# flanglet/kanzi-cpp

Hardware: AMD Instinct MI355X
Metric: encode+decode MB/s on the synthetic stand-in for silesia.tar (bit-exact) (higher is better)
Workload: dtype u8

## Files before the change

kanzi-cpp_amd/csrc/bwt_fwd.hip:

```cpp
#include "common.hpp"
#include "stages.hpp"
#include "bwt_common.hpp"

#include <cstdlib>
#include <cstring>
#include <algorithm>
#include <cmath>
#include "prims.hpp"
#include <chrono>
#include <vector>

namespace knz {

constexpr u32 SM_TS = 1792;
constexpr u32 SM_WIN = 2048;
constexpr u32 SM_G = 256;
constexpr u32 MED_CAP = 8192;
constexpr u32 SUPER_CAP = 8192;
constexpr int GATHER_THREADS = 512;
constexpr u32 GATHER_ROWS = 16;
static_assert(MED_CAP <= GATHER_ROWS * GATHER_THREADS, "k_bwt_f_gather_desc judges a medium group from one batch of loads");
constexpr u32 LARGE_OS_MIN = 1000000;
constexpr u32 NO_BIT = 0x7FFFFFFFu;

struct FwdView {
    const u32* base;
    int nBlocks;
    u32 total;
    u32* SA;
    u32* ISA;
    u64* ISA2;
    u32 round;
// ... 10 lines not shown

constexpr u32 VERDICT_WHOLE = 1, VERDICT_PLAIN = 2;
__host__ __device__ __forceinline__ u32 verdict_word(u32 round, u32 status, u32 members) { return (round << 24) | (status << 16) | members; }
static_assert(MED_CAP < (1u << 16), "verdict_word keeps a medium group's size in 16 bits");

enum FwdCounter : u32 {
    CNT_SMALL_LEFT = 0,
    CNT_MED = 1,
    CNT_LARGE = 2,
    CNT_LARGE_MEMBERS = 3,
    CNT_RUN = 4,
    CNT_RUN_MEMBERS = 5,
    CNT_RUN_LONGEST = 6,
    CNT_SUPER = 7,
    CNT_RUNS = 8,
    CNT_STAT_SMALL = 10,
    CNT_STAT_SMALL_GROUPS = 11,
    CNT_STAT_MED = 12,
    CNT_TIED = 13,
    CNT_PROBE_CAND = 14,
    CNT_LINKED = 14,
    CNT_LINK_TIED = 15,
    CNT_STAT_MED_GROUPS = 16,
    CNT_STAT_UNSPLIT = 17,
    CNT_STAT_UNSPLIT_MEMBERS = 18,
    CNT_STAT_MAJ = 19,
    CNT_STAT_MAJ_MEMBERS = 20,
    CNT_STAT_ASLEEP = 21,
    CNT_STAT_ASLEEP_MEMBERS = 22,
    CNT_ROUND_SLOTS = 24,
// ... 1114 lines not shown
        const u32 lab = (size <= SM_G) ? hdSlot : ((oldLab >= hdSlot && oldLab < hdSlot + size) ? oldLab : hdSlot + (size >> 1));
        (void)relO;
        const u32 gp = L.oV[t];
        v.SA[slot] = gp;
        if (lab != oldLab) lab_set(v, gp, L.blkBase, lab, oldLab);
        if (t == hd) {
            if (hdSlot != gs) atomicOr(&v.gnew[hdSlot >> 5], 1u << (hdSlot & 31));
            if (size > SM_G) v.medStage[hdSlot >> 8] = make_uint2(hdSlot, size);
            else if (size > 1) surv = 1;
        }
    }
    if (__ballot(surv != 0) != 0 && (tid & 63) == 0) v.counters[CNT_SMALL_LEFT] = 1;
}

template <int THREADS, int ROWS, bool STATS>
__global__ __launch_bounds__(THREADS, (THREADS >= 1024 ? 4 : THREADS / 128)) void k_bwt_f_sort_medium(FwdView v, const uint2* __restrict__ desc, u32 nDesc, int npass, u32 minLen,
                                                               uint2* __restrict__ medNext, uint2* __restrict__ largeNext, const uint2* __restrict__ descInfo,
                                                               uint4* __restrict__ superList)
{
    constexpr int WAVES = THREADS / 64;
    constexpr u32 CAP = (u32)ROWS * THREADS;
    __shared__ MedLds<THREADS, ROWS> L;
    const int tid = (int)threadIdx.x, lane = tid & 63, wave = tid >> 6;
    const unsigned long long ltMask = (lane == 0) ? 0ull : (~0ull >> (64 - lane));

    for (u32 g = blockIdx.x; g < nDesc; g += gridDim.x) {
        const uint2 d = desc[g];
        const u32 gs = d.x, n = d.y;
        if (n <= minLen || n > CAP) continue;
        const uint2 info = descInfo[g];
        {
            u32 k[ROWS], p[ROWS];
#pragma unroll
            for (int r = 0; r < ROWS; r++) { const u32 i = (u32)tid + (u32)r * THREADS; k[r] = 0; p[r] = 0; if (i < n) { k[r] = v.K[gs + i]; p[r] = v.SA[gs + i]; } }
#pragma unroll
            for (int r = 0; r < ROWS; r++) { const u32 i = (u32)tid + (u32)r * THREADS; if (i < n) { L.oK[i] = k[r]; L.oV[i] = p[r]; } }
        }
        __syncthreads();
        if (tid == 0) { L.oldLab = info.y; L.blkBase = info.x; }
        const u32 ka = L.oK[n >> 2], kb = L.oK[n >> 1], kc = L.oK[(n >> 2) * 3];
        const u32 m = (ka == kc) ? ka : kb;
        u32 c = 0;
        for (u32 i = (u32)tid; i < n; i += THREADS) c += (L.oK[i] == m) ? 1u : 0u;
        c = med_block_sum(L, c);
        if (c < n && 2 * c >= n && n <= SUPER_CAP && m == info.y - info.x + 1u) {
            if (tid == 0) { const u32 at = atomicAdd(&v.counters[CNT_SUPER], 1u); superList[at] = make_uint4(gs, n, info.x, info.y); }
            __syncthreads();
            continue;
        }
        if (STATS && tid == 0 && c == n) { atomicAdd(&v.counters[CNT_STAT_UNSPLIT], 1u); atomicAdd(&v.counters[CNT_STAT_UNSPLIT_MEMBERS], n); }
        if (c < n) {
            if (2 * c >= n) {
                const int R = (int)((n + THREADS - 1) / THREADS);
                const u32 waveBase = (u32)wave * (u32)R * 64u;
                u32 key[ROWS], val[ROWS], pos[ROWS];
                u32 runO = 0, runE = 0;
#pragma unroll
                for (int r = 0; r < ROWS; r++) {
                    key[r] = m; val[r] = 0; pos[r] = 0xFFFFFFFFu;
                    if (r < R) {
                        const u32 idx = waveBase + (u32)r * 64u + (u32)lane;
                        const bool valid = idx < n;
                        if (valid) { key[r] = L.oK[idx]; val[r] = L.oV[idx]; }
                        const bool oth = valid && key[r] != m, same = valid && key[r] == m;
                        const unsigned long long bo = __ballot(oth), be = __ballot(same);
                        if (oth) pos[r] = runO + (u32)__popcll(bo & ltMask);
                        if (same) pos[r] = 0x80000000u | (runE + (u32)__popcll(be & ltMask));
                        runO += (u32)__popcll(bo);
                        runE += (u32)__popcll(be);
                    }
                }
                if (lane == 0) { L.wtot[wave] = runO; L.wtot2[wave] = runE; }
                __syncthreads();
                u32 baseO = 0, baseE = 0, nOth = 0;
                for (int w = 0; w < WAVES; w++) { if (w < wave) { baseO += L.wtot[w]; baseE += L.wtot2[w]; } nOth += L.wtot[w]; }
#pragma unroll
                for (int r = 0; r < ROWS; r++) {
                    if (r < R && pos[r] != 0xFFFFFFFFu) {
                        const u32 at = (pos[r] & 0x80000000u) ? (nOth + baseE + (pos[r] & 0x7FFFFFFFu)) : (baseO + pos[r]);
                        L.oK[at] = key[r];
                        L.oV[at] = val[r];
                    }
                }
                __syncthreads();
                if (nOth <= (u32)THREADS) {
                    u32 kk = 0, vv = 0, at = 0;
                    if ((u32)tid < nOth) {
                        kk = L.oK[tid]; vv = L.oV[tid];
                        for (u32 j = 0; j < nOth; j++) { const u32 kj = L.oK[j]; at += (kj < kk || (kj == kk && j < (u32)tid)) ? 1u : 0u; }
                    }
                    __syncthreads();
                    if ((u32)tid < nOth) { L.oK[at] = kk; L.oV[at] = vv; }
                    __syncthreads();
                    u32 lessQ = 0;
                    if ((u32)tid < nOth) lessQ = (L.oK[tid] < m) ? 1u : 0u;
                    lessQ = med_block_sum(L, lessQ);
                    if (tid == 0) { L.oldLab = info.y; L.blkBase = info.x; if (STATS) { atomicAdd(&v.counters[CNT_STAT_MAJ], 1u); atomicAdd(&v.counters[CNT_STAT_MAJ_MEMBERS], n); } }
                    __syncthreads();
                    med_majority_write_back<THREADS, ROWS>(L, v, gs, n, nOth, c, lessQ, m);
                    __syncthreads();
                    continue;
                } else {
                    med_radix_sort<THREADS, ROWS>(L, nOth, npass);
                }
                u32 less = 0;
                for (u32 i = (u32)tid; i < nOth; i += THREADS) less += (L.oK[i] < m) ? 1u : 0u;
                less = med_block_sum(L, less);
#pragma unroll
                for (int k = 0; k < ROWS; k++) {
                    const u32 i = (u32)tid + (u32)k * THREADS;
                    if (i < n) { key[k] = L.oK[i]; val[k] = L.oV[i]; }
                }
                __syncthreads();
#pragma unroll
                for (int k = 0; k < ROWS; k++) {
                    const u32 i = (u32)tid + (u32)k * THREADS;
                    if (i < n) {
                        const u32 at = (i < less) ? i : (i < nOth ? i + c : less + (i - nOth));
                        L.oK[at] = key[k];
                        L.oV[at] = val[k];
                    }
                }
                __syncthreads();
            } else {
                med_radix_sort<THREADS, ROWS>(L, n, npass);
            }
        }
        med_write_back<THREADS, ROWS>(L, v, gs, n, medNext, largeNext);
        __syncthreads();
    }
}

__global__ __launch_bounds__(1024) void k_bwt_f_super(FwdView v, const uint4* __restrict__ superList, u32 h, int npass, uint2* __restrict__ medNext, uint2* __restrict__ largeNext)
{
    constexpr int THREADS = 1024, ROWS = 8;
    constexpr u32 CAP = (u32)ROWS * THREADS;
    __shared__ MedLds<THREADS, ROWS> L;
    __shared__ u16 nxt[CAP];
    __shared__ u16 cn[CAP];
    __shared__ u16 trEnd[CAP];
    __shared__ u32 sEnds;
    __shared__ u32 sMoved[2];
    __shared__ u32 sCmax;
    const int tid = (int)threadIdx.x, lane = tid & 63;
// ... 667 lines not shown
        const u32 step = ((u32)chunks * st == n) ? st : st + 1;
        const u32 logNbChunks = (u32)ilog2_u32((u32)chunks);
        d[0] = (u8)((logNbChunks << 2) | (pIndexSize - 1));
        u32 idx = 1;
        for (int k = 0; k < chunks; k++) {
            const u32 prim = lab_cur(fv, bb + (u32)k * step, bb) - bb;
            for (int sh = (int)(pIndexSize - 1) * 8; sh >= 0; sh -= 8) d[idx++] = (u8)(prim >> sh);
        }
        newLen[b] = hdr + n;
    }
}

__global__ __launch_bounds__(256) void k_bwt_f_med_flags(const uint2* __restrict__ stage, u32 nSlots, u32* __restrict__ flags)
{
    const u32 i = blockIdx.x * 256 + threadIdx.x;
    if (i < nSlots) flags[i] = stage[i].y ? 1u : 0u;
}

__global__ __launch_bounds__(256) void k_bwt_f_med_compact(uint2* __restrict__ stage, u32 nSlots, const u32* __restrict__ prefix, uint2* __restrict__ medNext)
{
    const u32 i = blockIdx.x * 256 + threadIdx.x;
    if (i >= nSlots) return;
    const uint2 d = stage[i];
    if (d.y) { medNext[prefix[i]] = d; stage[i] = make_uint2(0u, 0u); }
}

struct FwdTuning { int nsym; int noRunRound; int runFallback; int stats; int link; int plainLabels; int noPack; int noUnsplitSkip; int noGroupSleep; };
static FwdTuning& fwd_tuning()
{
    static FwdTuning t = [] {
        FwdTuning x; x.nsym = 0; x.noRunRound = 0; x.runFallback = 0; x.stats = 0; x.link = 1; x.plainLabels = 0; x.noPack = 0; x.noUnsplitSkip = 0; x.noGroupSleep = 0;
        if (getenv("KNZ_BWT_PLAIN_LABELS")) x.plainLabels = 1;
        if (getenv("KNZ_BWT_NO_PACK")) x.noPack = 1;
        if (getenv("KNZ_BWT_NO_UNSPLIT_SKIP")) x.noUnsplitSkip = 1;
        if (getenv("KNZ_BWT_NO_GROUP_SLEEP")) x.noGroupSleep = 1;
        if (const char* e = getenv("KNZ_BWT_LINK")) x.link = atoi(e);
        if (getenv("KNZ_BWT_STATS")) x.stats = 1;
        if (const char* e = getenv("KNZ_BWT_NSYM")) x.nsym = atoi(e);
        if (getenv("KNZ_BWT_NO_RUN_ROUND")) x.noRunRound = 1;
        if (getenv("KNZ_BWT_RUN_FALLBACK")) x.runFallback = 1;
        return x;
    }();
    return t;
}
int bwt_forward_tune(const char* key, int value)
{
    FwdTuning& t = fwd_tuning();
    if (!strcmp(key, "rs_onesweep")) { prims::rs_onesweep_knob().store(value); return 0; }
    if (!strcmp(key, "bwt_nsym")) t.nsym = value;
    else if (!strcmp(key, "bwt_no_run_round")) t.noRunRound = value;
    else if (!strcmp(key, "bwt_run_fallback")) t.runFallback = value;
    else if (!strcmp(key, "bwt_stats")) t.stats = value;
    else if (!strcmp(key, "bwt_link")) t.link = value;
    else if (!strcmp(key, "bwt_plain_labels")) t.plainLabels = value;
    else if (!strcmp(key, "bwt_no_pack")) t.noPack = value;
    else if (!strcmp(key, "bwt_no_unsplit_skip")) t.noUnsplitSkip = value;
    else if (!strcmp(key, "bwt_no_group_sleep")) t.noGroupSleep = value;
    else return -1;
    return 0;
}

struct FwdScratch {
    u64* keysA; u64* keysB;
    u32* valsA; u32* valsB;
    u32* SA; u32* ISA; u32* K; u64* ISA2;
    u32* t0; u32* t1; u32* t2; u32* t3;
    u32* gbits; u32* gnew; u32* rtbits; u32* ovr; size_t gbitsWords;
    uint2* med[2]; uint2* medStage; uint2* medVerdict[2]; u32* medFlags; u32* medPrefix; size_t medSlots; uint2* descInfo; uint2* large[2]; uint2* runList; uint4* superList; u32* ebits;
    u32* loff; u32* lbase;
    u32* survTile;
    u32* linkedTile;
    u32* base;
    u32* counters;
    u32* seg2;
    void* scanTmp;
    void* rsMem;
    u32* byteHist;
    u32* classTab; u32* rbits; u32* rcount; u32* rprefix;
    u32* runPos; u32* runE; u32* runL; u32* sE; u32* rcnt; u32* moff;
    u64* runKeysA; u64* runKeysB; u64* sKey;
    size_t maxRuns;
};

// ... 4 lines not shown
    u8* q = p;
    auto take = [&](size_t sz) { u8* r = q; q += fwd_align(sz); return r; };
    const size_t maxMed = 2 * (total / (SM_G + 1) + 2), maxLarge = total / (MED_CAP + 1) + 2;
    w->gbitsWords = ((total + 64) / 64 + SM_WIN / 64 + 4) * 2 + 128;
    w->keysA = (u64*)take(8 * total); w->keysB = (u64*)take(8 * total);
    w->valsA = (u32*)take(4 * total); w->valsB = (u32*)take(4 * total);
    w->SA = (u32*)take(4 * total); w->ISA = (u32*)take(4 * total); w->K = (u32*)take(4 * total);
    w->ISA2 = (VS <= (1u << LAB_BITS)) ? (u64*)take(8 * total) : (u64*)nullptr;
    w->t0 = (u32*)take(4 * total); w->t1 = (u32*)take(4 * total); w->t2 = (u32*)take(4 * total); w->t3 = (u32*)take(4 * total);
    w->gbits = (u32*)take(4 * w->gbitsWords);
    w->gnew = (u32*)take(4 * w->gbitsWords);
    w->rtbits = (u32*)take(4 * w->gbitsWords);
    w->ovr = (u32*)take(4 * total);
    w->med[0] = (uint2*)take(8 * maxMed); w->med[1] = (uint2*)take(8 * maxMed);
    w->medSlots = total / 256 + 2;
    w->medStage = (uint2*)take(8 * w->medSlots); w->medFlags = (u32*)take(4 * w->medSlots + 64); w->medPrefix = (u32*)take(4 * w->medSlots + 64);
    w->medVerdict[0] = (uint2*)take(16 * w->medSlots); w->medVerdict[1] = w->medVerdict[0] + w->medSlots;
    w->large[0] = (uint2*)take(8 * maxLarge); w->large[1] = (uint2*)take(8 * maxLarge);
    w->runList = (uint2*)take(8 * maxMed);
    w->superList = (uint4*)take(16 * maxMed);
    w->descInfo = (uint2*)take(8 * maxMed);
    w->ebits = (u32*)take(4 * w->gbitsWords);
    w->loff = (u32*)take(4 * (maxMed + 1));
    w->lbase = (u32*)take(4 * (maxMed + 1));
    w->survTile = (u32*)take(4 * (total / SM_TS + 64));
    w->linkedTile = (u32*)take(4 * (total / SM_TS + 64));
    w->base = (u32*)take(4ull * (nBlocks + 2));
    w->counters = (u32*)take(256);
    w->byteHist = (u32*)take(1024ull * (nBlocks + 1));
    w->seg2 = (u32*)take(64);
    w->scanTmp = take(prims::scan_tmp_bytes(total + 16));
// ... 33 lines not shown
        if (mode == UNTRIED && survMembers >= total / 8) { mode = TRIAL; trials++; return true; }
        if (mode == ON && survMembers >= total / 64) { mode = APPLIED; return true; }
        return false;
    }
};

struct FwdSort {
    hipStream_t s; const XfStage& st; u32* hp;
    const FwdTuning tune = fwd_tuning();
    BwtView bv; FwdView v; FwdScratch w; size_t maxTotal;
    prims::RsWs rs1;
    u32 total, medSlots, nTiles; int nsym, pbits, kbits;
    bool groupSleep = false;
    u32 h = 1; int cur = 0;
    u64 *keysFree, *keysFree2;
    u32 nRun, runElems, surv, nMed, nLarge, largeElems, survMembers;
    LinkPlan link; LinkTrial linkTr; std::chrono::steady_clock::time_point statT;
    int fetch(u32 first, u32 n) { return hipMemcpyAsync(hp + first, w.counters + first, 4 * (size_t)n, hipMemcpyDeviceToHost, s) == hipSuccess && hipStreamSynchronize(s) == hipSuccess ? 0 : -1; }
    void merge_bits() { hipLaunchKernelGGL(k_bwt_f_merge_bits, GRID1(total / 32 + 2), w.gbits, w.gnew, total / 32 + 2); }
    void enable_run_tiebits() { if (!v.rtbits) { hipMemsetAsync(w.rtbits, 0, 4 * w.gbitsWords, s); v.ovr = w.ovr; v.rtbits = w.rtbits; } }
    void compact_medium(uint2* dst)
    {
        KScope ks_("k_bwt_f_med_compact");
        hipLaunchKernelGGL(k_bwt_f_med_flags, GRID1(medSlots), w.medStage, medSlots, w.medFlags);
        prims::launch_scan<prims::SCAN_SUM_EXCL>(s, w.medFlags, w.medPrefix, medSlots, nullptr, w.scanTmp, w.counters + CNT_MED);
        hipLaunchKernelGGL(k_bwt_f_med_compact, GRID1(medSlots), w.medStage, medSlots, w.medPrefix, dst);
    }
    void bounds(u32 n, bool last, const u32* bits = nullptr, u32 len = 0, u32 wordsPerWin = 0)
    {
        if (bits) { KScope ks_("k_bwt_f_r0_winsum"); hipLaunchKernelGGL(k_bwt_f_r0_winsum, GRID1(n), bits, len, n, w.t0, w.t2, wordsPerWin); }
        if (last) { KScope ks_("k_bwt_f_scan_max"); prims::launch_scan<prims::SCAN_MAX_INCL>(s, w.t0, w.t1, n, nullptr, w.scanTmp); }
        KScope ks_("k_bwt_f_scan_min"); prims::launch_scan<prims::SCAN_MIN_INCL>(s, w.t2, w.t3, n, nullptr, w.scanTmp);
    }
    template <class KEY, bool HAS_VAL> int sort_one_segment(u32 n, KEY* ka, KEY* kb, u32* va, u32* vb, int loBit, int hiBit, bool oneRead = true)
    {
        hipLaunchKernelGGL(prims::k_rs_one_segment, dim3(1), dim3(64), 0, s, w.seg2, n);
        prims::rs_launch_layout(s, rs1);
        return prims::rs_sort<KEY, HAS_VAL>(s, rs1, ka, kb, va, vb, (size_t)n, loBit, hiBit, oneRead);
    }
    int setup(void* scratch, size_t scratchBytes, BwtSuffixArrays* sa)
    {
// ... 4 lines not shown
        hipMemsetAsync(st.newLen, 0, sizeof(u32) * st.nBlocks, s);
        { KScope ks_("k_bwt_f_r0_hist");
          hipMemsetAsync(w.byteHist, 0, 1024ull * st.nBlocks, s);
          hipLaunchKernelGGL(k_bwt_f_bytehist, dim3(64, (unsigned)st.nBlocks), dim3(256), 0, s, bv, w.base, w.byteHist);
          hipLaunchKernelGGL(k_bwt_f_choose_nsym, dim3(1), dim3(256), 0, s, w.byteHist, st.nBlocks, w.counters + CNT_LONGEST_BLOCK, w.counters + CNT_NSYM); }
        if (hipMemcpyAsync(hp, w.base + st.nBlocks, 4, hipMemcpyDeviceToHost, s) != hipSuccess || fetch(CNT_LONGEST_BLOCK, 2)) return -1;
        total = hp[0];
        if (sa) { sa->SA = w.SA; sa->base = w.base; sa->total = total; }
        if (total == 0) return 0;
        v.base = w.base; v.nBlocks = st.nBlocks; v.total = total; v.SA = w.SA; v.ISA = w.ISA; v.K = w.K; v.ISA2 = (w.ISA2 != nullptr && !tune.plainLabels) ? w.ISA2 : (u64*)nullptr;
        v.round = 0; v.gbits = w.gbits; v.gnew = w.gnew; v.counters = w.counters; v.medStage = w.medStage; v.ovr = nullptr; v.rtbits = nullptr;
        v.verdictNow = nullptr; v.verdictWas = nullptr;
        medSlots = (u32)((size_t)total / 256 + 1); nTiles = (total + SM_TS - 1) / SM_TS;
        survMembers = total;
        hipMemsetAsync(w.medStage, 0, 8ull * w.medSlots, s);
        groupSleep = !tune.noUnsplitSkip && !tune.noGroupSleep;
        if (groupSleep) hipMemsetAsync(w.medVerdict[0], 0, 16ull * w.medSlots, s);
        pbits = bits_for(hp[CNT_LONGEST_BLOCK], 1);
        const int fit = (64 - pbits) / 8, want = (hp[CNT_NSYM] == 5u) ? 5 : 4;
        nsym = fit < want ? fit : want;
        if (tune.nsym >= 1) nsym = tune.nsym < fit ? tune.nsym : fit;
        if (nsym < 1) return -4;
        while (2 * h <= (u32)nsym) h <<= 1;
        return 0;
    }
    void round0_sort()
    {
        const prims::RsWs rs = prims::rs_carve(w.rsMem, maxTotal, st.nBlocks + 1, w.base, st.nBlocks);
        rs1 = prims::rs_carve(w.rsMem, maxTotal, st.nBlocks + 1, w.seg2, 1);
        { KScope ks_("k_bwt_f_r0_layout"); prims::rs_launch_layout(s, rs); }
// ... 76 lines not shown
        bounds(nWinM, true, mbits, runElems, SM_WIN / 32);
        { KScope ks_("k_bwt_f_large_place");
          hipMemsetAsync(w.rtbits, 0, 4 * w.gbitsWords, s);
          hipLaunchKernelGGL(k_bwt_f_run_place, dim3((runElems + 255) / 256), dim3(256), 0, s, v, w.runList, w.loff, runElems, hbits + kbits, rk, rv, mbits, w.t1, w.t3, nWinM, w.large[cur],
                             w.valsB, w.ovr, w.rtbits, w.lbase);
          v.ovr = w.ovr; v.rtbits = w.rtbits; }
        { KScope ks_("k_bwt_f_merge_bits"); merge_bits(); }
        return 0;
    }
    int probe()
    {
        u32* probeCand = w.medFlags;
        compact_medium(w.med[cur]);
        { KScope ks_("k_bwt_f_probe"); hipLaunchKernelGGL(k_bwt_f_probe_scan, dim3(256), dim3(256), 0, s, v, w.med[cur], (u32)nsym, v.rtbits, probeCand); }
        if (fetch(0, CNT_ROUND_SLOTS)) return -1;
        surv = hp[CNT_SMALL_LEFT]; nMed = hp[CNT_MED]; nLarge = hp[CNT_LARGE]; largeElems = hp[CNT_LARGE_MEMBERS];
        if (const u32 nCand = hp[CNT_PROBE_CAND]) {
            enable_run_tiebits();
            hipMemsetAsync(w.counters, 0, 4 * CNT_PROBE_SLOTS, s);
            { KScope ks_("k_bwt_f_probe");
              hipLaunchKernelGGL(k_bwt_f_probe, dim3(std::min<u32>(nCand, 4096)), dim3(512), 0, s, bv, v, w.med[cur], probeCand, nCand, (u32)nsym, w.med[cur ^ 1], w.large[cur], w.ovr, w.rtbits);
              merge_bits(); }
            compact_medium(w.med[cur] + nMed);
            if (fetch(0, CNT_PROBE_SLOTS)) return -1;
            surv |= hp[CNT_SMALL_LEFT]; nMed += hp[CNT_MED];
        }
        if (tune.stats) fprintf(stderr, "after round 0 (nsym %d, total %u): run groups %u (%u members); small left %u, medium %u, large %u (%u members)\n",
                                nsym, total, nRun, runElems, surv, nMed, nLarge, largeElems);
        statT = std::chrono::steady_clock::now();
        return 0;
    }
    void link_step()
    {
        KScope ks_("k_bwt_f_link");
        u32* posflag = w.ebits; u32* linked = w.rbits; u32* rev = w.rcount; u32* sufRev = w.rprefix;
        const bool trial = link.mode == LinkPlan::TRIAL; linkTr.n = 0;
        if (trial) { linkTr.blk[linkTr.n++] = 0; if (st.nBlocks >= 5) linkTr.blk[linkTr.n++] = st.nBlocks / 2; if (st.nBlocks >= 3) linkTr.blk[linkTr.n++] = st.nBlocks - 1; }
        const u32 nW = total / 32 + 1;
        hipMemsetAsync(posflag, 0, 4 * (size_t)nW, s);
        hipMemsetAsync(linked, 0, 4 * ((size_t)nTiles * (SM_TS / 32) + 64), s);
// ... 6 lines not shown
        hipLaunchKernelGGL(k_bwt_f_link_apply, gridL, dim3(256), 0, s, v, posflag, sufRev, nW, linked, h, w.ovr, w.rtbits, 1u, linkTr);
    }
    void sort_small(bool linked)
    {
        KScope ks_("k_bwt_f_sort_small");
        u32* survTile = tune.link ? w.survTile : nullptr;
        if (v.ISA2 && pbits <= 23 && !tune.noPack) hipLaunchKernelGGL(k_bwt_f_small_fused<true>, dim3(nTiles), dim3(256), 0, s, v, h, survTile, tune.stats);
        else if (v.ISA2) hipLaunchKernelGGL(k_bwt_f_small_fused<false>, dim3(nTiles), dim3(256), 0, s, v, h, survTile, tune.stats);
        else hipLaunchKernelGGL(k_bwt_f_sort_small, dim3(nTiles), dim3(256), 0, s, v, survTile);
        if (linked) hipLaunchKernelGGL(k_bwt_f_link_payoff, dim3(1), dim3(256), 0, s, v, w.linkedTile, w.survTile, nTiles, 1u, w.counters + CNT_LINKED, linkTr);
        if (tune.link) prims::launch_scan<prims::SCAN_SUM_EXCL>(s, w.survTile, w.survTile, nTiles, nullptr, w.scanTmp, w.counters + CNT_TIED);
    }
    void sort_medium()
    {
        const int npass = (kbits + 7) / 8, nxt = cur ^ 1;
        { KScope ks_("k_bwt_f_sort_medium"); const dim3 gridM(std::min<u32>(nMed, 8192));
          const auto sort256 = tune.stats ? k_bwt_f_sort_medium<256, 8, true> : k_bwt_f_sort_medium<256, 8, false>;
          const auto sort512 = tune.stats ? k_bwt_f_sort_medium<512, 16, true> : k_bwt_f_sort_medium<512, 16, false>;
          hipLaunchKernelGGL(sort256, gridM, dim3(256), 0, s, v, w.med[cur], nMed, npass, SM_G, w.med[nxt], w.large[nxt], w.descInfo, w.superList);
          hipLaunchKernelGGL(sort512, gridM, dim3(512), 0, s, v, w.med[cur], nMed, npass, 2048u, w.med[nxt], w.large[nxt], w.descInfo, w.superList); }
        { KScope ks_("k_bwt_f_super"); hipLaunchKernelGGL(k_bwt_f_super, dim3(std::min<u32>(nMed, 512)), dim3(1024), 0, s, v, w.superList, h, npass, w.med[nxt], w.large[nxt]); }
    }
    template <class KEY> void large_keys()
    {
        { KScope ks_("k_bwt_f_large_prefix"); hipLaunchKernelGGL(k_bwt_f_large_prefix, dim3(1), dim3(1024), 0, s, w.large[cur], nLarge, w.loff, w.base, st.nBlocks, w.lbase); }
        KScope ks_("k_bwt_f_large_keys");
        hipLaunchKernelGGL(k_bwt_f_large_keys<KEY>, GRID1(largeElems), v, w.large[cur], nLarge, w.loff, largeElems, h, kbits, reinterpret_cast<KEY*>(keysFree), w.valsA);
    }
    template <class KEY> void sort_large(int lbits)
    {
        KEY* ka = reinterpret_cast<KEY*>(keysFree); KEY* kb = reinterpret_cast<KEY*>(keysFree2); int r;
        { KScope ks_("k_bwt_f_sort_large");
          r = sort_one_segment<KEY, true>(largeElems, ka, kb, w.valsA, w.valsB, 0, kbits + lbits, largeElems >= LARGE_OS_MIN); }
        const KEY* sk = r ? kb : ka; const u32* sv = r ? w.valsB : w.valsA;
        { KScope ks_("k_bwt_f_large_flags"); hipLaunchKernelGGL(k_bwt_f_large_flags<KEY>, GRID1(largeElems), sk, largeElems, w.t0, w.t2); }
        bounds(largeElems, true);
        { KScope ks_("k_bwt_f_large_place");
          hipLaunchKernelGGL(k_bwt_f_large_place<KEY>, GRID1(largeElems), v, w.large[cur], w.loff, largeElems, kbits, sk, sv, w.t1, w.t3, w.med[cur ^ 1], w.large[cur ^ 1], w.lbase); }
    }
    int end_round()
    {
        { KScope ks_("k_bwt_f_merge_bits"); merge_bits(); }
        compact_medium(w.med[cur ^ 1]);
        if (fetch(0, CNT_ROUND_SLOTS)) return -1;
        surv = hp[CNT_SMALL_LEFT]; nMed = hp[CNT_MED]; nLarge = hp[CNT_LARGE]; largeElems = hp[CNT_LARGE_MEMBERS]; survMembers = hp[CNT_TIED];
        if (tune.stats) {
            std::vector<u32> hs(nTiles); u32 activeTiles = 0;
            if (tune.link && hipMemcpyAsync(hs.data(), w.survTile, 4 * (size_t)nTiles, hipMemcpyDeviceToHost, s) == hipSuccess && hipStreamSynchronize(s) == hipSuccess) {
                for (u32 t = 0; t + 1 < nTiles; t++) activeTiles += hs[t + 1] != hs[t] ? 1u : 0u;
                fprintf(stderr, "  windows with tied small groups after the round: %u of %u\n", activeTiles, nTiles);
            }
            const std::chrono::steady_clock::time_point now = std::chrono::steady_clock::now();
            fprintf(stderr, "round h=%u (%.3f ms): small members worked on %u in %u groups, medium members %u; after it: small left %u, medium groups %u, large %u (%u members); %u groups took the chain round; %u small members still tied\n",
                    h, std::chrono::duration<double, std::milli>(now - statT).count(), hp[CNT_STAT_SMALL], hp[CNT_STAT_SMALL_GROUPS], hp[CNT_STAT_MED], surv, nMed, nLarge, largeElems,
                    hp[CNT_SUPER], hp[CNT_TIED]);
            fprintf(stderr, "  medium groups worked on %u (%u members): all keys equal in %u (%u members)%s, majority path %u (%u members), asleep %u (%u members)\n", hp[CNT_STAT_MED_GROUPS], hp[CNT_STAT_MED],
                    hp[CNT_STAT_UNSPLIT], hp[CNT_STAT_UNSPLIT_MEMBERS], tune.noUnsplitSkip ? "" : " -- left alone", hp[CNT_STAT_MAJ], hp[CNT_STAT_MAJ_MEMBERS], hp[CNT_STAT_ASLEEP], hp[CNT_STAT_ASLEEP_MEMBERS]);
            statT = now;
        }
        cur ^= 1; h <<= 1;
        return 0;
    }
    int round()
    {
        if (h > bv.VS) return -5;
        { KScope ks_("k_bwt_f_round"); hipMemsetAsync(w.counters, 0, 4 * CNT_ROUND_SLOTS, s); }
        if (++v.round > 255) return -5;
        const bool linked = surv && tune.link && h >= (u32)(tune.link > 1 ? tune.link : 32)
                            && link.next(h, survMembers, total, hp[CNT_LINKED], hp[CNT_LINK_TIED], tune.stats);
        if (linked) link_step();
        if (surv && !v.ISA2) { KScope ks_("k_bwt_f_gather_small"); hipLaunchKernelGGL(k_bwt_f_gather_small, dim3(nTiles), dim3(256), 0, s, v, h, tune.stats); }
        if (groupSleep) { v.verdictNow = w.medVerdict[v.round & 1]; v.verdictWas = w.medVerdict[(v.round & 1) ^ 1]; }
        if (groupSleep && nMed && v.round >= 2) { KScope ks_("k_bwt_f_med_sleep"); hipLaunchKernelGGL(k_bwt_f_med_sleep, GRID1(nMed), v, w.med[cur], nMed, tune.stats); }
        if (nMed) { KScope ks_("k_bwt_f_gather_desc"); hipLaunchKernelGGL(k_bwt_f_gather_desc, dim3(1024), dim3(GATHER_THREADS), 0, s, v, w.med[cur], nMed, h, w.descInfo, tune.stats, tune.noUnsplitSkip ? 0 : 1); }
        const int lbits = bits_for(nLarge, 0); const bool key32 = kbits + lbits <= 32;
        if (nLarge) { if (key32) large_keys<u32>(); else large_keys<u64>(); }
        if (surv) sort_small(linked);
        if (nMed) sort_medium();
        if (nLarge) { if (key32) sort_large<u32>(lbits); else sort_large<u64>(lbits); }
        return end_round();
    }
    void emit()
    {
        KScope ks_("k_bwt_f_emit");
        hipLaunchKernelGGL(k_bwt_f_emit, dim3((unsigned)std::min<size_t>(((size_t)bv.VS + 255) / 256, 4096), st.nBlocks), dim3(256), 0, s, bv, w.base, st.ok, w.SA, v, st.newLen);
    }
};

static int bwt_forward_run(hipStream_t s, const XfStage& st, void* scratch, size_t scratchBytes, u32* h_pinned, BwtSuffixArrays* sa)
// ... 18 lines not shown
```

Measured before the change: 6680.

## Fuse medium-group key gather into the medium sort kernel, split groups by size

Adds a fused kernel that gathers each medium group's keys directly into registers and LDS, judges unsplit groups, and sorts them in one pass. This removes the separate gather_desc kernel and its global write and re-read of K. The compaction step now also partitions medium groups into small and large size-class index lists, so each list launches with a suitably sized block and the grid is spread across XCDs. The fused path only runs when ISA2 is present. The existing sort logic is moved into a shared device function, and the fused kernel adds per-group find_block work.

```diff
diff --git a/kanzi-cpp_amd/csrc/bwt_fwd.hip b/kanzi-cpp_amd/csrc/bwt_fwd.hip
--- a/kanzi-cpp_amd/csrc/bwt_fwd.hip
+++ b/kanzi-cpp_amd/csrc/bwt_fwd.hip
@@ -16,6 +16,7 @@
 constexpr u32 SM_WIN = 2048;
 constexpr u32 SM_G = 256;
 constexpr u32 MED_CAP = 8192;
+constexpr u32 MED_LO_CAP = 2048;
 constexpr u32 SUPER_CAP = 8192;
 constexpr int GATHER_THREADS = 512;
 constexpr u32 GATHER_ROWS = 16;
@@ -56,6 +57,7 @@
     CNT_RUN_LONGEST = 6,
     CNT_SUPER = 7,
     CNT_RUNS = 8,
+    CNT_MED_LO = 9,
     CNT_STAT_SMALL = 10,
     CNT_STAT_SMALL_GROUPS = 11,
     CNT_STAT_MED = 12,
@@ -1200,15 +1202,114 @@
 }
 
 template <int THREADS, int ROWS, bool STATS>
+__device__ __forceinline__ void med_sort_group(MedLds<THREADS, ROWS>& L, const FwdView& v, u32 gs, u32 n, uint2 info, int npass, bool storeKeys,
+                                               uint2* __restrict__ medNext, uint2* __restrict__ largeNext, uint4* __restrict__ superList)
+{
+    constexpr int WAVES = THREADS / 64;
+    const int tid = (int)threadIdx.x, lane = tid & 63, wave = tid >> 6;
+    const unsigned long long ltMask = (lane == 0) ? 0ull : (~0ull >> (64 - lane));
+    if (tid == 0) { L.oldLab = info.y; L.blkBase = info.x; }
+    const u32 ka = L.oK[n >> 2], kb = L.oK[n >> 1], kc = L.oK[(n >> 2) * 3];
+    const u32 m = (ka == kc) ? ka : kb;
+    u32 c = 0;
+    for (u32 i = (u32)tid; i < n; i += THREADS) c += (L.oK[i] == m) ? 1u : 0u;
+    c = med_block_sum(L, c);
+    if (c < n && 2 * c >= n && n <= SUPER_CAP && m == info.y - info.x + 1u) {
+        if (tid == 0) { const u32 at = atomicAdd(&v.counters[CNT_SUPER], 1u); superList[at] = make_uint4(gs, n, info.x, info.y); }
+        if (storeKeys) for (u32 i = (u32)tid; i < n; i += THREADS) v.K[gs + i] = L.oK[i];
+        __syncthreads();
+        return;
+    }
+    if (STATS && tid == 0 && c == n) { atomicAdd(&v.counters[CNT_STAT_UNSPLIT], 1u); atomicAdd(&v.counters[CNT_STAT_UNSPLIT_MEMBERS], n); }
+    if (c < n) {
+        if (2 * c >= n) {
+            const int R = (int)((n + THREADS - 1) / THREADS);
+            const u32 waveBase = (u32)wave * (u32)R * 64u;
+            u32 key[ROWS], val[ROWS], pos[ROWS];
+            u32 runO = 0, runE = 0;
+#pragma unroll
+            for (int r = 0; r < ROWS; r++) {
+                key[r] = m; val[r] = 0; pos[r] = 0xFFFFFFFFu;
+                if (r < R) {
+                    const u32 idx = waveBase + (u32)r * 64u + (u32)lane;
+                    const bool valid = idx < n;
+                    if (valid) { key[r] = L.oK[idx]; val[r] = L.oV[idx]; }
+                    const bool oth = valid && key[r] != m, same = valid && key[r] == m;
+                    const unsigned long long bo = __ballot(oth), be = __ballot(same);
+                    if (oth) pos[r] = runO + (u32)__popcll(bo & ltMask);
+                    if (same) pos[r] = 0x80000000u | (runE + (u32)__popcll(be & ltMask));
+                    runO += (u32)__popcll(bo);
+                    runE += (u32)__popcll(be);
+                }
+            }
+            if (lane == 0) { L.wtot[wave] = runO; L.wtot2[wave] = runE; }
+            __syncthreads();
+            u32 baseO = 0, baseE = 0, nOth = 0;
+            for (int w = 0; w < WAVES; w++) { if (w < wave) { baseO += L.wtot[w]; baseE += L.wtot2[w]; } nOth += L.wtot[w]; }
+#pragma unroll
+            for (int r = 0; r < ROWS; r++) {
+                if (r < R && pos[r] != 0xFFFFFFFFu) {
+                    const u32 at = (pos[r] & 0x80000000u) ? (nOth + baseE + (pos[r] & 0x7FFFFFFFu)) : (baseO + pos[r]);
+                    L.oK[at] = key[r];
+                    L.oV[at] = val[r];
+                }
+            }
+            __syncthreads();
+            if (nOth <= (u32)THREADS) {
+                u32 kk = 0, vv = 0, at = 0;
+                if ((u32)tid < nOth) {
+                    kk = L.oK[tid]; vv = L.oV[tid];
+                    for (u32 j = 0; j < nOth; j++) { const u32 kj = L.oK[j]; at += (kj < kk || (kj == kk && j < (u32)tid)) ? 1u : 0u; }
+                }
+                __syncthreads();
+                if ((u32)tid < nOth) { L.oK[at] = kk; L.oV[at] = vv; }
+                __syncthreads();
+                u32 lessQ = 0;
+                if ((u32)tid < nOth) lessQ = (L.oK[tid] < m) ? 1u : 0u;
+                lessQ = med_block_sum(L, lessQ);
+                if (tid == 0) { L.oldLab = info.y; L.blkBase = info.x; if (STATS) { atomicAdd(&v.counters[CNT_STAT_MAJ], 1u); atomicAdd(&v.counters[CNT_STAT_MAJ_MEMBERS], n); } }
+                __syncthreads();
+                med_majority_write_back<THREADS, ROWS>(L, v, gs, n, nOth, c, lessQ, m);
+                __syncthreads();
+                return;
+            } else {
+                med_radix_sort<THREADS, ROWS>(L, nOth, npass);
+            }
+            u32 less = 0;
+            for (u32 i = (u32)tid; i < nOth; i += THREADS) less += (L.oK[i] < m) ? 1u : 0u;
+            less = med_block_sum(L, less);
+#pragma unroll
+            for (int k = 0; k < ROWS; k++) {
+                const u32 i = (u32)tid + (u32)k * THREADS;
+                if (i < n) { key[k] = L.oK[i]; val[k] = L.oV[i]; }
+            }
+            __syncthreads();
+#pragma unroll
+            for (int k = 0; k < ROWS; k++) {
+                const u32 i = (u32)tid + (u32)k * THREADS;
+                if (i < n) {
+                    const u32 at = (i < less) ? i : (i < nOth ? i + c : less + (i - nOth));
+                    L.oK[at] = key[k];
+                    L.oV[at] = val[k];
+                }
+            }
+            __syncthreads();
+        } else {
+            med_radix_sort<THREADS, ROWS>(L, n, npass);
+        }
+    }
+    med_write_back<THREADS, ROWS>(L, v, gs, n, medNext, largeNext);
+    __syncthreads();
+}
+
+template <int THREADS, int ROWS, bool STATS>
 __global__ __launch_bounds__(THREADS, (THREADS >= 1024 ? 4 : THREADS / 128)) void k_bwt_f_sort_medium(FwdView v, const uint2* __restrict__ desc, u32 nDesc, int npass, u32 minLen,
                                                                uint2* __restrict__ medNext, uint2* __restrict__ largeNext, const uint2* __restrict__ descInfo,
                                                                uint4* __restrict__ superList)
 {
-    constexpr int WAVES = THREADS / 64;
     constexpr u32 CAP = (u32)ROWS * THREADS;
     __shared__ MedLds<THREADS, ROWS> L;
-    const int tid = (int)threadIdx.x, lane = tid & 63, wave = tid >> 6;
-    const unsigned long long ltMask = (lane == 0) ? 0ull : (~0ull >> (64 - lane));
+    const int tid = (int)threadIdx.x;
 
     for (u32 g = blockIdx.x; g < nDesc; g += gridDim.x) {
         const uint2 d = desc[g];
@@ -1223,97 +1324,64 @@
             for (int r = 0; r < ROWS; r++) { const u32 i = (u32)tid + (u32)r * THREADS; if (i < n) { L.oK[i] = k[r]; L.oV[i] = p[r]; } }
         }
         __syncthreads();
-        if (tid == 0) { L.oldLab = info.y; L.blkBase = info.x; }
-        const u32 ka = L.oK[n >> 2], kb = L.oK[n >> 1], kc = L.oK[(n >> 2) * 3];
-        const u32 m = (ka == kc) ? ka : kb;
-        u32 c = 0;
-        for (u32 i = (u32)tid; i < n; i += THREADS) c += (L.oK[i] == m) ? 1u : 0u;
-        c = med_block_sum(L, c);
-        if (c < n && 2 * c >= n && n <= SUPER_CAP && m == info.y - info.x + 1u) {
-            if (tid == 0) { const u32 at = atomicAdd(&v.counters[CNT_SUPER], 1u); superList[at] = make_uint4(gs, n, info.x, info.y); }
+        med_sort_group<THREADS, ROWS, STATS>(L, v, gs, n, info, npass, false, medNext, largeNext, superList);
+    }
+}
+
+template <int THREADS, int ROWS, bool STATS>
+__global__ __launch_bounds__(THREADS, 4) void k_bwt_f_medium_fused(FwdView v, const uint2* __restrict__ desc, const u32* __restrict__ classIdx, u32 nClass, u32 h, int npass,
+                                                               int skip, uint2* __restrict__ medNext, uint2* __restrict__ largeNext, uint4* __restrict__ superList)
+{
+    constexpr u32 CAP = (u32)ROWS * THREADS;
+    __shared__ MedLds<THREADS, ROWS> L;
+    __shared__ u32 sDiff;
+    const int tid = (int)threadIdx.x;
+    const u32 xcd = blockIdx.x & 7, lanesPerXcd = gridDim.x >> 3, slot = blockIdx.x >> 3;
+    const u32 per = (nClass + 7) / 8;
+    const u32 lo = xcd * per, hi = (lo + per < nClass) ? lo + per : nClass;
+    if (tid == 0) sDiff = 0;
+    __syncthreads();
+    for (u32 g = lo + slot; g < hi; g += lanesPerXcd) {
+        const uint2 d = desc[classIdx[g]];
+        const u32 gs = d.x, n = d.y;
+        if (n <= SM_G || n > CAP) continue;
+        const int blk = find_block(v.base, v.nBlocks, gs);
+        const u32 bb = v.base[blk], be = v.base[blk + 1];
+        u32 off = h;
+        if (v.rtbits && ((v.rtbits[gs >> 5] >> (gs & 31)) & 1u)) { const u32 r = v.ovr[gs]; off = r > h ? r : h; }
+        const u32 gp0 = v.SA[gs];
+        const u32 lab = lab_old(v, gp0, bb), key0 = gather_key(v, gp0, off, bb, be);
+        const bool judge = skip && lab - gs < n;
+        u32 gp[ROWS], key[ROWS];
+#pragma unroll
+        for (int r = 0; r < ROWS; r++) { const u32 i = (u32)tid + (u32)r * THREADS; gp[r] = (i < n) ? v.SA[gs + i] : bb; }
+#pragma unroll
+        for (int r = 0; r < ROWS; r++) { const u32 i = (u32)tid + (u32)r * THREADS; key[r] = (i < n) ? gather_key(v, gp[r], off, bb, be) : key0; }
+        bool unsplit = false;
+        if (judge) {
+            bool diff = false;
+#pragma unroll
+            for (int r = 0; r < ROWS; r++) diff = diff || key[r] != key0;
+            if (__ballot(diff) != 0 && (tid & 63) == 0) sDiff = 1;
             __syncthreads();
-            continue;
-        }
-        if (STATS && tid == 0 && c == n) { atomicAdd(&v.counters[CNT_STAT_UNSPLIT], 1u); atomicAdd(&v.counters[CNT_STAT_UNSPLIT_MEMBERS], n); }
-        if (c < n) {
-            if (2 * c >= n) {
-                const int R = (int)((n + THREADS - 1) / THREADS);
-                const u32 waveBase = (u32)wave * (u32)R * 64u;
-                u32 key[ROWS], val[ROWS], pos[ROWS];
-                u32 runO = 0, runE = 0;
-#pragma unroll
-                for (int r = 0; r < ROWS; r++) {
-                    key[r] = m; val[r] = 0; pos[r] = 0xFFFFFFFFu;
-                    if (r < R) {
-                        const u32 idx = waveBase + (u32)r * 64u + (u32)lane;
-                        const bool valid = idx < n;
-                        if (valid) { key[r] = L.oK[idx]; val[r] = L.oV[idx]; }
-                        const bool oth = valid && key[r] != m, same = valid && key[r] == m;
-                        const unsigned long long bo = __ballot(oth), be = __ballot(same);
-                        if (oth) pos[r] = runO + (u32)__popcll(bo & ltMask);
-                        if (same) pos[r] = 0x80000000u | (runE + (u32)__popcll(be & ltMask));
-                        runO += (u32)__popcll(bo);
-                        runE += (u32)__popcll(be);
-                    }
-                }
-                if (lane == 0) { L.wtot[wave] = runO; L.wtot2[wave] = runE; }
-                __syncthreads();
-                u32 baseO = 0, baseE = 0, nOth = 0;
-                for (int w = 0; w < WAVES; w++) { if (w < wave) { baseO += L.wtot[w]; baseE += L.wtot2[w]; } nOth += L.wtot[w]; }
-#pragma unroll
-                for (int r = 0; r < ROWS; r++) {
-                    if (r < R && pos[r] != 0xFFFFFFFFu) {
-                        const u32 at = (pos[r] & 0x80000000u) ? (nOth + baseE + (pos[r] & 0x7FFFFFFFu)) : (baseO + pos[r]);
-                        L.oK[at] = key[r];
-                        L.oV[at] = val[r];
-                    }
-                }
-                __syncthreads();
-                if (nOth <= (u32)THREADS) {
-                    u32 kk = 0, vv = 0, at = 0;
-                    if ((u32)tid < nOth) {
-                        kk = L.oK[tid]; vv = L.oV[tid];
-                        for (u32 j = 0; j < nOth; j++) { const u32 kj = L.oK[j]; at += (kj < kk || (kj == kk && j < (u32)tid)) ? 1u : 0u; }
-                    }
-                    __syncthreads();
-                    if ((u32)tid < nOth) { L.oK[at] = kk; L.oV[at] = vv; }
-                    __syncthreads();
-                    u32 lessQ = 0;
-                    if ((u32)tid < nOth) lessQ = (L.oK[tid] < m) ? 1u : 0u;
-                    lessQ = med_block_sum(L, lessQ);
-                    if (tid == 0) { L.oldLab = info.y; L.blkBase = info.x; if (STATS) { atomicAdd(&v.counters[CNT_STAT_MAJ], 1u); atomicAdd(&v.counters[CNT_STAT_MAJ_MEMBERS], n); } }
-                    __syncthreads();
-                    med_majority_write_back<THREADS, ROWS>(L, v, gs, n, nOth, c, lessQ, m);
-                    __syncthreads();
-                    continue;
-                } else {
-                    med_radix_sort<THREADS, ROWS>(L, nOth, npass);
-                }
-                u32 less = 0;
-                for (u32 i = (u32)tid; i < nOth; i += THREADS) less += (L.oK[i] < m) ? 1u : 0u;
-                less = med_block_sum(L, less);
-#pragma unroll
-                for (int k = 0; k < ROWS; k++) {
-                    const u32 i = (u32)tid + (u32)k * THREADS;
-                    if (i < n) { key[k] = L.oK[i]; val[k] = L.oV[i]; }
-                }
-                __syncthreads();
-#pragma unroll
-                for (int k = 0; k < ROWS; k++) {
-                    const u32 i = (u32)tid + (u32)k * THREADS;
-                    if (i < n) {
-                        const u32 at = (i < less) ? i : (i < nOth ? i + c : less + (i - nOth));
-                        L.oK[at] = key[k];
-                        L.oV[at] = val[k];
-                    }
-                }
-                __syncthreads();
-            } else {
-                med_radix_sort<THREADS, ROWS>(L, n, npass);
+            unsplit = sDiff == 0;
+        }
+        if (tid == 0) {
+            if (unsplit) {
+                v.medStage[gs >> 8] = d;
+                if (v.verdictNow) v.verdictNow[gs >> 8] = make_uint2(key0, verdict_word(v.round, (off == h && key0 != 0u) ? VERDICT_PLAIN : VERDICT_WHOLE, n));
             }
-        }
-        med_write_back<THREADS, ROWS>(L, v, gs, n, medNext, largeNext);
-        __syncthreads();
+            if (STATS) {
+                atomicAdd(&v.counters[CNT_STAT_MED], n); atomicAdd(&v.counters[CNT_STAT_MED_GROUPS], 1u);
+                if (unsplit) { atomicAdd(&v.counters[CNT_STAT_UNSPLIT], 1u); atomicAdd(&v.counters[CNT_STAT_UNSPLIT_MEMBERS], n); }
+            }
+        }
+        if (unsplit) { __syncthreads(); continue; }
+#pragma unroll
+        for (int r = 0; r < ROWS; r++) { const u32 i = (u32)tid + (u32)r * THREADS; if (i < n) { L.oK[i] = key[r]; L.oV[i] = gp[r]; } }
+        __syncthreads();
+        if (tid == 0) sDiff = 0;
+        med_sort_group<THREADS, ROWS, STATS>(L, v, gs, n, make_uint2(bb, lab), npass, true, medNext, largeNext, superList);
     }
 }
 
@@ -2011,26 +2079,36 @@
 __global__ __launch_bounds__(256) void k_bwt_f_med_flags(const uint2* __restrict__ stage, u32 nSlots, u32* __restrict__ flags)
 {
     const u32 i = blockIdx.x * 256 + threadIdx.x;
-    if (i < nSlots) flags[i] = stage[i].y ? 1u : 0u;
-}
-
-__global__ __launch_bounds__(256) void k_bwt_f_med_compact(uint2* __restrict__ stage, u32 nSlots, const u32* __restrict__ prefix, uint2* __restrict__ medNext)
+    if (i >= nSlots) return;
+    const u32 n = stage[i].y;
+    flags[i] = (n != 0 && n <= MED_LO_CAP) ? 1u : 0u;
+    flags[nSlots + i] = (n > MED_LO_CAP) ? 1u : 0u;
+}
+
+__global__ __launch_bounds__(256) void k_bwt_f_med_compact(uint2* __restrict__ stage, u32 nSlots, const u32* __restrict__ prefix, uint2* __restrict__ medNext,
+                                                           u32 at, u32* __restrict__ idxLo, u32 atLo, u32* __restrict__ idxHi, u32 atHi, u32* __restrict__ nLoOut)
 {
     const u32 i = blockIdx.x * 256 + threadIdx.x;
     if (i >= nSlots) return;
+    const u32 nLo = prefix[nSlots];
+    if (i == 0) *nLoOut = nLo;
     const uint2 d = stage[i];
-    if (d.y) { medNext[prefix[i]] = d; stage[i] = make_uint2(0u, 0u); }
-}
-
-struct FwdTuning { int nsym; int noRunRound; int runFallback; int stats; int link; int plainLabels; int noPack; int noUnsplitSkip; int noGroupSleep; };
+    if (d.y == 0) return;
+    const u32 pLo = prefix[i], pHi = prefix[nSlots + i] - nLo, g = at + pLo + pHi;
+    medNext[g] = d; stage[i] = make_uint2(0u, 0u);
+    if (d.y <= MED_LO_CAP) idxLo[atLo + pLo] = g; else idxHi[atHi + pHi] = g;
+}
+
+struct FwdTuning { int nsym; int noRunRound; int runFallback; int stats; int link; int plainLabels; int noPack; int noUnsplitSkip; int noGroupSleep; int noMediumFuse; };
 static FwdTuning& fwd_tuning()
 {
     static FwdTuning t = [] {
-        FwdTuning x; x.nsym = 0; x.noRunRound = 0; x.runFallback = 0; x.stats = 0; x.link = 1; x.plainLabels = 0; x.noPack = 0; x.noUnsplitSkip = 0; x.noGroupSleep = 0;
+        FwdTuning x; x.nsym = 0; x.noRunRound = 0; x.runFallback = 0; x.stats = 0; x.link = 1; x.plainLabels = 0; x.noPack = 0; x.noUnsplitSkip = 0; x.noGroupSleep = 0; x.noMediumFuse = 0;
         if (getenv("KNZ_BWT_PLAIN_LABELS")) x.plainLabels = 1;
         if (getenv("KNZ_BWT_NO_PACK")) x.noPack = 1;
         if (getenv("KNZ_BWT_NO_UNSPLIT_SKIP")) x.noUnsplitSkip = 1;
         if (getenv("KNZ_BWT_NO_GROUP_SLEEP")) x.noGroupSleep = 1;
+        if (getenv("KNZ_BWT_NO_MEDIUM_FUSE")) x.noMediumFuse = 1;
         if (const char* e = getenv("KNZ_BWT_LINK")) x.link = atoi(e);
         if (getenv("KNZ_BWT_STATS")) x.stats = 1;
         if (const char* e = getenv("KNZ_BWT_NSYM")) x.nsym = atoi(e);
@@ -2053,6 +2131,7 @@
     else if (!strcmp(key, "bwt_no_pack")) t.noPack = value;
     else if (!strcmp(key, "bwt_no_unsplit_skip")) t.noUnsplitSkip = value;
     else if (!strcmp(key, "bwt_no_group_sleep")) t.noGroupSleep = value;
+    else if (!strcmp(key, "bwt_no_medium_fuse")) t.noMediumFuse = value;
     else return -1;
     return 0;
 }
@@ -2063,7 +2142,7 @@
     u32* SA; u32* ISA; u32* K; u64* ISA2;
     u32* t0; u32* t1; u32* t2; u32* t3;
     u32* gbits; u32* gnew; u32* rtbits; u32* ovr; size_t gbitsWords;
-    uint2* med[2]; uint2* medStage; uint2* medVerdict[2]; u32* medFlags; u32* medPrefix; size_t medSlots; uint2* descInfo; uint2* large[2]; uint2* runList; uint4* superList; u32* ebits;
+    uint2* med[2]; uint2* medStage; uint2* medVerdict[2]; u32* medFlags; u32* medPrefix; u32* medIdxLo; u32* medIdxHi; size_t medSlots; uint2* descInfo; uint2* large[2]; uint2* runList; uint4* superList; u32* ebits;
     u32* loff; u32* lbase;
     u32* survTile;
     u32* linkedTile;
@@ -2098,7 +2177,8 @@
     w->ovr = (u32*)take(4 * total);
     w->med[0] = (uint2*)take(8 * maxMed); w->med[1] = (uint2*)take(8 * maxMed);
     w->medSlots = total / 256 + 2;
-    w->medStage = (uint2*)take(8 * w->medSlots); w->medFlags = (u32*)take(4 * w->medSlots + 64); w->medPrefix = (u32*)take(4 * w->medSlots + 64);
+    w->medStage = (uint2*)take(8 * w->medSlots); w->medFlags = (u32*)take(8 * w->medSlots + 64); w->medPrefix = (u32*)take(8 * w->medSlots + 64);
+    w->medIdxLo = (u32*)take(4 * maxMed); w->medIdxHi = (u32*)take(4 * maxMed);
     w->medVerdict[0] = (uint2*)take(16 * w->medSlots); w->medVerdict[1] = w->medVerdict[0] + w->medSlots;
     w->large[0] = (uint2*)take(8 * maxLarge); w->large[1] = (uint2*)take(8 * maxLarge);
     w->runList = (uint2*)take(8 * maxMed);
@@ -2162,17 +2242,19 @@
     bool groupSleep = false;
     u32 h = 1; int cur = 0;
     u64 *keysFree, *keysFree2;
+    bool medFuse = false;
+    u32 nMedLo = 0;
     u32 nRun, runElems, surv, nMed, nLarge, largeElems, survMembers;
     LinkPlan link; LinkTrial linkTr; std::chrono::steady_clock::time_point statT;
     int fetch(u32 first, u32 n) { return hipMemcpyAsync(hp + first, w.counters + first, 4 * (size_t)n, hipMemcpyDeviceToHost, s) == hipSuccess && hipStreamSynchronize(s) == hipSuccess ? 0 : -1; }
     void merge_bits() { hipLaunchKernelGGL(k_bwt_f_merge_bits, GRID1(total / 32 + 2), w.gbits, w.gnew, total / 32 + 2); }
     void enable_run_tiebits() { if (!v.rtbits) { hipMemsetAsync(w.rtbits, 0, 4 * w.gbitsWords, s); v.ovr = w.ovr; v.rtbits = w.rtbits; } }
-    void compact_medium(uint2* dst)
+    void compact_medium(uint2* dst, u32 at = 0, u32 atLo = 0)
     {
         KScope ks_("k_bwt_f_med_compact");
         hipLaunchKernelGGL(k_bwt_f_med_flags, GRID1(medSlots), w.medStage, medSlots, w.medFlags);
-        prims::launch_scan<prims::SCAN_SUM_EXCL>(s, w.medFlags, w.medPrefix, medSlots, nullptr, w.scanTmp, w.counters + CNT_MED);
-        hipLaunchKernelGGL(k_bwt_f_med_compact, GRID1(medSlots), w.medStage, medSlots, w.medPrefix, dst);
+        prims::launch_scan<prims::SCAN_SUM_EXCL>(s, w.medFlags, w.medPrefix, 2 * (size_t)medSlots, nullptr, w.scanTmp, w.counters + CNT_MED);
+        hipLaunchKernelGGL(k_bwt_f_med_compact, GRID1(medSlots), w.medStage, medSlots, w.medPrefix, dst, at, w.medIdxLo, atLo, w.medIdxHi, at - atLo, w.counters + CNT_MED_LO);
     }
     void bounds(u32 n, bool last, const u32* bits = nullptr, u32 len = 0, u32 wordsPerWin = 0)
     {
@@ -2207,6 +2289,7 @@
         medSlots = (u32)((size_t)total / 256 + 1); nTiles = (total + SM_TS - 1) / SM_TS;
         survMembers = total;
         hipMemsetAsync(w.medStage, 0, 8ull * w.medSlots, s);
+        medFuse = v.ISA2 != nullptr && !tune.noMediumFuse;
         groupSleep = !tune.noUnsplitSkip && !tune.noGroupSleep;
         if (groupSleep) hipMemsetAsync(w.medVerdict[0], 0, 16ull * w.medSlots, s);
         pbits = bits_for(hp[CNT_LONGEST_BLOCK], 1);
@@ -2313,16 +2396,16 @@
         compact_medium(w.med[cur]);
         { KScope ks_("k_bwt_f_probe"); hipLaunchKernelGGL(k_bwt_f_probe_scan, dim3(256), dim3(256), 0, s, v, w.med[cur], (u32)nsym, v.rtbits, probeCand); }
         if (fetch(0, CNT_ROUND_SLOTS)) return -1;
-        surv = hp[CNT_SMALL_LEFT]; nMed = hp[CNT_MED]; nLarge = hp[CNT_LARGE]; largeElems = hp[CNT_LARGE_MEMBERS];
+        surv = hp[CNT_SMALL_LEFT]; nMed = hp[CNT_MED]; nMedLo = hp[CNT_MED_LO]; nLarge = hp[CNT_LARGE]; largeElems = hp[CNT_LARGE_MEMBERS];
         if (const u32 nCand = hp[CNT_PROBE_CAND]) {
             enable_run_tiebits();
             hipMemsetAsync(w.counters, 0, 4 * CNT_PROBE_SLOTS, s);
             { KScope ks_("k_bwt_f_probe");
               hipLaunchKernelGGL(k_bwt_f_probe, dim3(std::min<u32>(nCand, 4096)), dim3(512), 0, s, bv, v, w.med[cur], probeCand, nCand, (u32)nsym, w.med[cur ^ 1], w.large[cur], w.ovr, w.rtbits);
               merge_bits(); }
-            compact_medium(w.med[cur] + nMed);
-            if (fetch(0, CNT_PROBE_SLOTS)) return -1;
-            surv |= hp[CNT_SMALL_LEFT]; nMed += hp[CNT_MED];
+            compact_medium(w.med[cur], nMed, nMedLo);
+            if (fetch(0, CNT_MED_LO + 1)) return -1;
+            surv |= hp[CNT_SMALL_LEFT]; nMed += hp[CNT_MED]; nMedLo += hp[CNT_MED_LO];
         }
         if (tune.stats) fprintf(stderr, "after round 0 (nsym %d, total %u): run groups %u (%u members); small left %u, medium %u, large %u (%u members)\n",
                                 nsym, total, nRun, runElems, surv, nMed, nLarge, largeElems);
@@ -2359,11 +2442,17 @@
     void sort_medium()
     {
         const int npass = (kbits + 7) / 8, nxt = cur ^ 1;
-        { KScope ks_("k_bwt_f_sort_medium"); const dim3 gridM(std::min<u32>(nMed, 8192));
+        if (medFuse) {
+            KScope ks_("k_bwt_f_medium_fused"); const int skip = tune.noUnsplitSkip ? 0 : 1; const u32 nMedHi = nMed - nMedLo;
+            const auto fuse256 = tune.stats ? k_bwt_f_medium_fused<256, 8, true> : k_bwt_f_medium_fused<256, 8, false>;
+            const auto fuse512 = tune.stats ? k_bwt_f_medium_fused<512, 16, true> : k_bwt_f_medium_fused<512, 16, false>;
+            if (nMedLo) hipLaunchKernelGGL(fuse256, dim3(std::min<u32>((nMedLo + 7) / 8 * 8, 2048)), dim3(256), 0, s, v, w.med[cur], w.medIdxLo, nMedLo, h, npass, skip, w.med[nxt], w.large[nxt], w.superList);
+            if (nMedHi) hipLaunchKernelGGL(fuse512, dim3(std::min<u32>((nMedHi + 7) / 8 * 8, 1024)), dim3(512), 0, s, v, w.med[cur], w.medIdxHi, nMedHi, h, npass, skip, w.med[nxt], w.large[nxt], w.superList);
+        } else { KScope ks_("k_bwt_f_sort_medium"); const dim3 gridM(std::min<u32>(nMed, 8192));
           const auto sort256 = tune.stats ? k_bwt_f_sort_medium<256, 8, true> : k_bwt_f_sort_medium<256, 8, false>;
           const auto sort512 = tune.stats ? k_bwt_f_sort_medium<512, 16, true> : k_bwt_f_sort_medium<512, 16, false>;
           hipLaunchKernelGGL(sort256, gridM, dim3(256), 0, s, v, w.med[cur], nMed, npass, SM_G, w.med[nxt], w.large[nxt], w.descInfo, w.superList);
-          hipLaunchKernelGGL(sort512, gridM, dim3(512), 0, s, v, w.med[cur], nMed, npass, 2048u, w.med[nxt], w.large[nxt], w.descInfo, w.superList); }
+          hipLaunchKernelGGL(sort512, gridM, dim3(512), 0, s, v, w.med[cur], nMed, npass, MED_LO_CAP, w.med[nxt], w.large[nxt], w.descInfo, w.superList); }
         { KScope ks_("k_bwt_f_super"); hipLaunchKernelGGL(k_bwt_f_super, dim3(std::min<u32>(nMed, 512)), dim3(1024), 0, s, v, w.superList, h, npass, w.med[nxt], w.large[nxt]); }
     }
     template <class KEY> void large_keys()
@@ -2388,7 +2477,7 @@
         { KScope ks_("k_bwt_f_merge_bits"); merge_bits(); }
         compact_medium(w.med[cur ^ 1]);
         if (fetch(0, CNT_ROUND_SLOTS)) return -1;
-        surv = hp[CNT_SMALL_LEFT]; nMed = hp[CNT_MED]; nLarge = hp[CNT_LARGE]; largeElems = hp[CNT_LARGE_MEMBERS]; survMembers = hp[CNT_TIED];
+        surv = hp[CNT_SMALL_LEFT]; nMed = hp[CNT_MED]; nMedLo = hp[CNT_MED_LO]; nLarge = hp[CNT_LARGE]; largeElems = hp[CNT_LARGE_MEMBERS]; survMembers = hp[CNT_TIED];
         if (tune.stats) {
             std::vector<u32> hs(nTiles); u32 activeTiles = 0;
             if (tune.link && hipMemcpyAsync(hs.data(), w.survTile, 4 * (size_t)nTiles, hipMemcpyDeviceToHost, s) == hipSuccess && hipStreamSynchronize(s) == hipSuccess) {
@@ -2417,7 +2506,7 @@
         if (surv && !v.ISA2) { KScope ks_("k_bwt_f_gather_small"); hipLaunchKernelGGL(k_bwt_f_gather_small, dim3(nTiles), dim3(256), 0, s, v, h, tune.stats); }
         if (groupSleep) { v.verdictNow = w.medVerdict[v.round & 1]; v.verdictWas = w.medVerdict[(v.round & 1) ^ 1]; }
         if (groupSleep && nMed && v.round >= 2) { KScope ks_("k_bwt_f_med_sleep"); hipLaunchKernelGGL(k_bwt_f_med_sleep, GRID1(nMed), v, w.med[cur], nMed, tune.stats); }
-        if (nMed) { KScope ks_("k_bwt_f_gather_desc"); hipLaunchKernelGGL(k_bwt_f_gather_desc, dim3(1024), dim3(GATHER_THREADS), 0, s, v, w.med[cur], nMed, h, w.descInfo, tune.stats, tune.noUnsplitSkip ? 0 : 1); }
+        if (nMed && !medFuse) { KScope ks_("k_bwt_f_gather_desc"); hipLaunchKernelGGL(k_bwt_f_gather_desc, dim3(1024), dim3(GATHER_THREADS), 0, s, v, w.med[cur], nMed, h, w.descInfo, tune.stats, tune.noUnsplitSkip ? 0 : 1); }
         const int lbits = bits_for(nLarge, 0); const bool key32 = kbits + lbits <= 32;
         if (nLarge) { if (key32) large_keys<u32>(); else large_keys<u64>(); }
         if (surv) sort_small(linked);
```

After: 6878 (median of 6 runs). 3.0% higher.
